# MooreThreads/LiteGS

Measured on NVIDIA H100. Metric: forward+backward views/sec @1080p 1M Gaussians, higher is better.
Workload: dtype f32

## Files before the change

### litegs_b200/csrc/sort.cu

```cuda
#include <cub/device/device_radix_sort.cuh>
#include <cub/block/block_scan.cuh>
#include <algorithm>
#include <cstdlib>
#include <cstring>
#include "common.cuh"

namespace {

constexpr int RS_THREADS = 256;
constexpr int RS_WARPS = RS_THREADS / 32;
constexpr int RS_MAXBINS = 256;

int g_sort_impl = -1;
bool g_sort_forced = false;

int sort_impl()
{
    if (g_sort_impl < 0) {
        const char* e = getenv("LGS_SORT");
        g_sort_forced = e != nullptr;
        g_sort_impl = (e != nullptr && strcmp(e, "cub") == 0) ? 0 : 1;
    }
    return g_sort_impl;
}
// ... 31 lines not shown
#pragma unroll
    for (int k = 0; k < RS_WARPS; k++) h[k][t] = 0;
    __syncthreads();
    const unsigned mask = (unsigned)nbins - 1u;
    int* hw = h[w];
    if (VEC && base + TILE <= n) {
        const uint4* v = reinterpret_cast<const uint4*>(keys + base);
#pragma unroll
        for (int j = 0; j < IPT / KPV; j++) {
            uint4 q = v[j * RS_THREADS + t];
            unsigned x[4] = { q.x, q.y, q.z, q.w };
#pragma unroll
            for (int c = 0; c < 4; c++) {
                if (sizeof(KeyT) == 2) {
                    atomicAdd(&hw[(((x[c] & 0xffffu) - bias) >> shift) & mask], 1);
                    atomicAdd(&hw[(((x[c] >> 16) - bias) >> shift) & mask], 1);
                } else {
                    atomicAdd(&hw[((x[c] - bias) >> shift) & mask], 1);
                }
            }
        }
    } else {
#pragma unroll
        for (int i = 0; i < IPT; i++) {
            int idx = base + i * RS_THREADS + t;
            if (idx < n) atomicAdd(&hw[(((unsigned)keys[idx] - bias) >> shift) & mask], 1);
        }
    }
    __syncthreads();
    if (t < nbins) {
        int c = 0;
#pragma unroll
        for (int k = 0; k < RS_WARPS; k++) c += h[k][t];
        table[(size_t)t * nblocks + blockIdx.x] = c;
    }
}

__global__ void __launch_bounds__(RS_THREADS) rs_scan_rows_kernel(int* __restrict__ table, int nblocks, int* __restrict__ totals)
{
    using BlockScan = cub::BlockScan<int, RS_THREADS>;
    __shared__ typename BlockScan::TempStorage s_scan;
    int* row = table + (size_t)blockIdx.x * nblocks;
    const int per = (nblocks + RS_THREADS - 1) / RS_THREADS;
    const int lo = min(nblocks, (int)threadIdx.x * per), hi = min(nblocks, lo + per);
    int sum = 0;
    for (int k = lo; k < hi; k++) sum += row[k];
    int pre, tot;
    BlockScan(s_scan).ExclusiveSum(sum, pre, tot);
    for (int k = lo; k < hi; k++) { int c = row[k]; row[k] = pre; pre += c; }
    if (threadIdx.x == 0) totals[blockIdx.x] = tot;
}

template <typename KeyT, int IPT, int NS>
__global__ void __launch_bounds__(RS_THREADS, IPT == 16 ? 3 : 4) rs_scatter_kernel(const KeyT* __restrict__ kin, const unsigned* __restrict__ vin,
                                                                KeyT* __restrict__ kout, unsigned* __restrict__ vout, int n, int shift,
                                                                int nbins, int nblocks, const int* __restrict__ table,
                                                                const int* __restrict__ totals, unsigned bias,
                                                                const int* __restrict__ n_dev, const unsigned* __restrict__ bias_dev)
{
    constexpr int TILE = RS_THREADS * IPT;
    static_assert(IPT % NS == 0, "the ranking rounds must tile the items of a lane");
    if (n_dev != nullptr) n = min(n, max(*n_dev, 0));
    if (bias_dev != nullptr) bias = *bias_dev;
    if ((int)blockIdx.x * TILE >= n) return;
    using BlockScan = cub::BlockScan<int, RS_THREADS>;
    __shared__ int s_cnt[RS_WARPS][RS_MAXBINS];
    __shared__ int s_gofs[RS_MAXBINS];
    __shared__ KeyT s_k[TILE];
    __shared__ unsigned s_v[TILE];
    unsigned* s_match = s_v;
    __shared__ typename BlockScan::TempStorage s_scan;
    const int t = threadIdx.x, lane = t & 31, w = t >> 5;
    const int base = blockIdx.x * TILE;
    const int nvalid = min(TILE, n - base);
    const unsigned mask = (unsigned)nbins - 1u;
    const unsigned lt = lanemask_lt();
#pragma unroll
    for (int k = 0; k < RS_WARPS; k++) s_cnt[k][t] = 0;
    for (int k = t; k < NS * RS_WARPS * nbins; k += RS_THREADS) s_match[k] = 0u;
    KeyT key[IPT];
    unsigned val[IPT];
    unsigned short rank[IPT];
#pragma unroll
    for (int i = 0; i < IPT; i++) {
        int loc = w * 32 * IPT + i * 32 + lane;
        bool valid = loc < nvalid;
        key[i] = valid ? kin[base + loc] : (KeyT)(bias - 1u);
        val[i] = valid ? vin[base + loc] : 0u;
    }
    int gdig;
    {
        int tot_d = t < nbins ? totals[t] : 0;
        BlockScan(s_scan).ExclusiveSum(tot_d, gdig);
        if (t < nbins) gdig += table[(size_t)t * nblocks + blockIdx.x];
    }
    __syncthreads();
    unsigned* mw = s_match + w * nbins;
    const int set_stride = RS_WARPS * nbins;
#pragma unroll
    for (int i0 = 0; i0 < IPT; i0 += NS) {
        unsigned d[NS];
#pragma unroll
        for (int q = 0; q < NS; q++) {
            d[q] = (((unsigned)key[i0 + q] - bias) >> shift) & mask;
            atomicOr(&mw[q * set_stride + d[q]], 1u << lane);
        }
        __syncwarp();
        unsigned own[NS];
#pragma unroll
        for (int j = 0; j < NS; j++) {
            int r = s_cnt[w][d[j]];
#pragma unroll
            for (int q = 0; q < j; q++) r += __popc(mw[q * set_stride + d[j]]);
            own[j] = mw[j * set_stride + d[j]];
            rank[i0 + j] = (unsigned short)(r + __popc(own[j] & lt));
        }
        __syncwarp();
#pragma unroll
        for (int j = 0; j < NS; j++) {
            if ((own[j] >> lane) <= 1u) {
                if (NS == 1) s_cnt[w][d[j]] = (int)rank[i0 + j] + 1;
                else atomicAdd(&s_cnt[w][d[j]], __popc(own[j]));
                mw[j * set_stride + d[j]] = 0u;
            }
        }
        __syncwarp();
    }
    __syncthreads();
    int tot = 0;
#pragma unroll
    for (int k = 0; k < RS_WARPS; k++) { int c = s_cnt[k][t]; s_cnt[k][t] = tot; tot += c; }
    int dbase;
    BlockScan(s_scan).ExclusiveSum(tot, dbase);
#pragma unroll
    for (int k = 0; k < RS_WARPS; k++) s_cnt[k][t] += dbase;
    s_gofs[t] = gdig - dbase;
    __syncthreads();
#pragma unroll
    for (int i = 0; i < IPT; i++) {
        unsigned d = (((unsigned)key[i] - bias) >> shift) & mask;
        int p = s_cnt[w][d] + rank[i];
        s_k[p] = key[i];
        s_v[p] = val[i];
    }
    __syncthreads();
#pragma unroll
    for (int i = 0; i < IPT; i++) {
        int k = i * RS_THREADS + t;
        if (k < nvalid) {
            KeyT kk = s_k[k];
            int dst = s_gofs[(((unsigned)kk - bias) >> shift) & mask] + k;
            kout[dst] = kk;
            vout[dst] = s_v[k];
        }
    }
}

constexpr unsigned LB_AGG = 1u << 30, LB_INC = 2u << 30, LB_MASK = (1u << 30) - 1u;
constexpr int RS_MAXPASS = 4;

struct GhistArgs { int shift[RS_MAXPASS]; int nbins[RS_MAXPASS]; int passes; };

template <typename KeyT, int IPT>
__global__ void __launch_bounds__(RS_THREADS) rs_ghist_kernel(const KeyT* __restrict__ keys, int n, GhistArgs A, int* __restrict__ ghist,
                                                              unsigned bias, const int* __restrict__ n_dev,
                                                              const unsigned* __restrict__ bias_dev)
{
    constexpr int TILE = RS_THREADS * IPT;
    __shared__ int h[RS_MAXPASS][RS_MAXBINS];
    const int t = threadIdx.x;
    if (n_dev != nullptr) n = min(n, max(*n_dev, 0));
    if (bias_dev != nullptr) bias = *bias_dev;
    const int base = blockIdx.x * TILE;
    if (base >= n) return;
    for (int p = 0; p < A.passes; p++) h[p][t] = 0;
    __syncthreads();
#pragma unroll
    for (int i = 0; i < IPT; i++) {
        const int idx = base + i * RS_THREADS + t;
        if (idx < n) {
            const unsigned k = (unsigned)keys[idx] - bias;
            for (int p = 0; p < A.passes; p++) atomicAdd(&h[p][(k >> A.shift[p]) & (unsigned)(A.nbins[p] - 1)], 1);
        }
    }
    __syncthreads();
    for (int p = 0; p < A.passes; p++)
        if (t < A.nbins[p] && h[p][t] != 0) atomicAdd(&ghist[p * RS_MAXBINS + t], h[p][t]);
}

template <typename KeyT, int IPT>
__global__ void __launch_bounds__(RS_THREADS) rs_onesweep_kernel(const KeyT* __restrict__ kin, const unsigned* __restrict__ vin,
                                                                 KeyT* __restrict__ kout, unsigned* __restrict__ vout, int n, int shift,
                                                                 int nbins, const int* __restrict__ ghist ,
                                                                 unsigned* __restrict__ status ,
                                                                 int* __restrict__ ticket, unsigned bias, const int* __restrict__ n_dev,
                                                                 const unsigned* __restrict__ bias_dev)
{
    constexpr int TILE = RS_THREADS * IPT;
    using BlockScan = cub::BlockScan<int, RS_THREADS>;
    __shared__ int s_cnt[RS_WARPS][RS_MAXBINS];
    __shared__ int s_gofs[RS_MAXBINS];
    __shared__ KeyT s_k[TILE];
    __shared__ unsigned s_v[TILE];
    __shared__ int s_tile;
    static_assert(TILE >= RS_WARPS * RS_MAXBINS, "the match slots alias the value staging buffer");
    unsigned (*s_match)[RS_MAXBINS] = reinterpret_cast<unsigned (*)[RS_MAXBINS]>(s_v);
    __shared__ typename BlockScan::TempStorage s_scan;
    const int t = threadIdx.x, lane = t & 31, w = t >> 5;
    if (n_dev != nullptr) n = min(n, max(*n_dev, 0));
    if (bias_dev != nullptr) bias = *bias_dev;
    if (t == 0) s_tile = atomicAdd(ticket, 1);
#pragma unroll
    for (int k = 0; k < RS_WARPS; k++) { s_cnt[k][t] = 0; s_match[k][t] = 0u; }
    __syncthreads();
    const int tile = s_tile;
    const int base = tile * TILE;
    if (base >= n) return;
    const int nvalid = min(TILE, n - base);
    const unsigned mask = (unsigned)nbins - 1u;
    const unsigned lt = lanemask_lt();
    KeyT key[IPT];
    unsigned val[IPT];
    unsigned short rank[IPT];
#pragma unroll
    for (int i = 0; i < IPT; i++) {
        int loc = w * 32 * IPT + i * 32 + lane;
        bool valid = loc < nvalid;
        key[i] = valid ? kin[base + loc] : (KeyT)(bias - 1u);
        val[i] = valid ? vin[base + loc] : 0u;
    }
    int gdig;
    {
        int tot_d = t < nbins ? ghist[t] : 0;
        BlockScan(s_scan).ExclusiveSum(tot_d, gdig);
    }
    __syncthreads();
#pragma unroll
    for (int i = 0; i < IPT; i++) {
        unsigned d = (((unsigned)key[i] - bias) >> shift) & mask;
        atomicOr(&s_match[w][d], 1u << lane);
        __syncwarp();
        unsigned m = s_match[w][d];
        int r = s_cnt[w][d] + __popc(m & lt);
        rank[i] = (unsigned short)r;
        __syncwarp();
        if ((m >> lane) <= 1u) { s_cnt[w][d] = r + 1; s_match[w][d] = 0u; }
        __syncwarp();
    }
    __syncthreads();
    int tot = 0;
#pragma unroll
    for (int k = 0; k < RS_WARPS; k++) { int c = s_cnt[k][t]; s_cnt[k][t] = tot; tot += c; }
    int real = tot;
    if (t == (int)mask) real -= (TILE - nvalid);
    if (t < nbins) {
        volatile unsigned* st_ = status + (size_t)tile * nbins;
        st_[t] = LB_AGG | (unsigned)real;
        unsigned prefix = 0u;
        for (int i = tile - 1; i >= 0;) {
            const unsigned v = *((volatile unsigned*)(status + (size_t)i * nbins + t));
            const unsigned flag = v & ~LB_MASK;
            if (flag == 0u) continue;
            prefix += v & LB_MASK;
            if (flag == LB_INC) break;
            i--;
        }
        st_[t] = LB_INC | (prefix + (unsigned)real);
        gdig += (int)prefix;
    }
    int dbase;
    BlockScan(s_scan).ExclusiveSum(tot, dbase);
#pragma unroll
    for (int k = 0; k < RS_WARPS; k++) s_cnt[k][t] += dbase;
    s_gofs[t] = gdig - dbase;
    __syncthreads();
#pragma unroll
    for (int i = 0; i < IPT; i++) {
        unsigned d = (((unsigned)key[i] - bias) >> shift) & mask;
        int p = s_cnt[w][d] + rank[i];
        s_k[p] = key[i];
        s_v[p] = val[i];
    }
    __syncthreads();
#pragma unroll
    for (int i = 0; i < IPT; i++) {
        int k = i * RS_THREADS + t;
        if (k < nvalid) {
            KeyT kk = s_k[k];
            int dst = s_gofs[(((unsigned)kk - bias) >> shift) & mask] + k;
            kout[dst] = kk;
            vout[dst] = s_v[k];
        }
    }
}

struct RsPlan {
    int ipt, tile, nblocks, passes, dbits;
    size_t table_bytes, scan_bytes, total_bytes, off_scan, off_keys, off_vals;
};

inline size_t align256(size_t x) { return (x + 255) & ~(size_t)255; }

template <typename KeyT>
RsPlan rs_plan(int n, int begin_bit, int end_bit)
{
    RsPlan p;
    static const int forced_ipt = getenv("LGS_RS_IPT") ? atoi(getenv("LGS_RS_IPT")) : 0;
    p.ipt = (forced_ipt == 8 || forced_ipt == 16) ? forced_ipt : (n > (1 << 22) ? 16 : 8);
    p.tile = RS_THREADS * p.ipt;
    p.nblocks = (n + p.tile - 1) / p.tile;
    int bits = end_bit - begin_bit;
    p.passes = bits <= 0 ? 0 : (bits + 7) / 8;
    p.dbits = p.passes == 0 ? 0 : (bits + p.passes - 1) / p.passes;
    p.table_bytes = align256((size_t)RS_MAXPASS * RS_MAXBINS * p.nblocks * sizeof(int));
    p.scan_bytes = align256((RS_MAXPASS * RS_MAXBINS + 64) * sizeof(int));
    p.off_scan = p.table_bytes;
    p.off_keys = p.off_scan + p.scan_bytes;
    p.off_vals = p.off_keys + align256((size_t)n * sizeof(KeyT));
    p.total_bytes = p.off_vals + align256((size_t)n * sizeof(unsigned));
    return p;
}

bool rs_use_onesweep();
template <typename KeyT>
int rs_sort_onesweep(const KeyT* keys_in, KeyT* keys_out, const unsigned* vals_in, unsigned* vals_out, int n, int begin_bit, int end_bit,
                     unsigned bias, char* ws, cudaStream_t st, const int* n_dev, const unsigned* bias_dev);

template <typename KeyT>
int rs_sort(const KeyT* keys_in, KeyT* keys_out, const unsigned* vals_in, unsigned* vals_out, int n, int begin_bit, int end_bit,
            unsigned bias, char* ws, cudaStream_t st, const int* n_dev = nullptr, const unsigned* bias_dev = nullptr)
{
    RsPlan p = rs_plan<KeyT>(n, begin_bit, end_bit);
    if (p.passes == 0) {
        LGS_REQUIRE(n_dev == nullptr, "sort_pairs: a device-side count needs at least one pass");
        LGS_CUDA(cudaMemcpyAsync(keys_out, keys_in, (size_t)n * sizeof(KeyT), cudaMemcpyDeviceToDevice, st));
        LGS_CUDA(cudaMemcpyAsync(vals_out, vals_in, (size_t)n * sizeof(unsigned), cudaMemcpyDeviceToDevice, st));
        return LGS_OK;
    }
    if (rs_use_onesweep())
        return rs_sort_onesweep<KeyT>(keys_in, keys_out, vals_in, vals_out, n, begin_bit, end_bit, bias, ws, st, n_dev, bias_dev);
    int* table = (int*)ws;
    int* totals = (int*)(ws + p.off_scan);
    KeyT* ktmp = (KeyT*)(ws + p.off_keys);
    unsigned* vtmp = (unsigned*)(ws + p.off_vals);
    const KeyT* ksrc = keys_in;
    const unsigned* vsrc = vals_in;
    int bit = begin_bit;
    for (int pass = 0; pass < p.passes; pass++) {
        int dbits = min(p.dbits, end_bit - bit);
        int nbins = 1 << dbits;
        bool to_out = ((p.passes - 1 - pass) & 1) == 0;
        KeyT* kdst = to_out ? keys_out : ktmp;
        unsigned* vdst = to_out ? vals_out : vtmp;
        const bool vec = ((uintptr_t)ksrc & 15) == 0;
        lgs_with_flags([&](auto ipt16, auto v) {
            rs_hist_kernel<KeyT, ipt16 ? 16 : 8, v><<<p.nblocks, RS_THREADS, 0, st>>>(ksrc, n, bit, nbins, p.nblocks, table, bias, n_dev,
                                                                                     bias_dev);
            return LGS_OK;
        }, p.ipt == 16, vec);
        LGS_CHECK_LAUNCH("rs_hist_kernel");
        rs_scan_rows_kernel<<<nbins, RS_THREADS, 0, st>>>(table, p.nblocks, totals);
        LGS_CHECK_LAUNCH("rs_scan_rows_kernel");
        static const int rank_cap = getenv("LGS_RS_RANK") ? atoi(getenv("LGS_RS_RANK")) : 2;
        int ns = 1;
        while (ns < 4 && ns * 2 <= rank_cap && ns * 2 * RS_WARPS * nbins <= p.tile) ns *= 2;
        lgs_with_flags([&](auto ipt16, auto ns4, auto ns2) {
            rs_scatter_kernel<KeyT, ipt16 ? 16 : 8, ns4 ? 4 : ns2 ? 2 : 1><<<p.nblocks, RS_THREADS, 0, st>>>(
                ksrc, vsrc, kdst, vdst, n, bit, nbins, p.nblocks, table, totals, bias, n_dev, bias_dev);
            return LGS_OK;
        }, p.ipt == 16, ns == 4, ns == 2);
        LGS_CHECK_LAUNCH("rs_scatter_kernel");
        ksrc = kdst; vsrc = vdst;
        bit += dbits;
    }
    return LGS_OK;
}

int g_rs_onesweep = -1;
bool rs_use_onesweep()
{
    if (g_rs_onesweep < 0) {
        const char* e = getenv("LGS_RS");
        g_rs_onesweep = (e != nullptr && e[0] == 'o') ? 1 : 0;
    }
    return g_rs_onesweep == 1;
}

template <typename KeyT>
int rs_sort_onesweep(const KeyT* keys_in, KeyT* keys_out, const unsigned* vals_in, unsigned* vals_out, int n, int begin_bit, int end_bit,
                     unsigned bias, char* ws, cudaStream_t st, const int* n_dev, const unsigned* bias_dev)
{
    RsPlan p = rs_plan<KeyT>(n, begin_bit, end_bit);
    unsigned* status = (unsigned*)ws;
    int* ghist = (int*)(ws + p.off_scan);
    int* tickets = ghist + RS_MAXPASS * RS_MAXBINS;
    KeyT* ktmp = (KeyT*)(ws + p.off_keys);
    unsigned* vtmp = (unsigned*)(ws + p.off_vals);
    GhistArgs A;
    A.passes = p.passes;
    size_t status_words = 0;
    int bit = begin_bit;
    for (int pass = 0; pass < p.passes; pass++) {
        int dbits = min(p.dbits, end_bit - bit);
        A.shift[pass] = bit; A.nbins[pass] = 1 << dbits;
        status_words += (size_t)p.nblocks * A.nbins[pass];
        bit += dbits;
    }
    LGS_CUDA(cudaMemsetAsync(status, 0, status_words * sizeof(unsigned), st));
    LGS_CUDA(cudaMemsetAsync(ghist, 0, (RS_MAXPASS * RS_MAXBINS + 64) * sizeof(int), st));
    lgs_with_flags([&](auto ipt16) {
        rs_ghist_kernel<KeyT, ipt16 ? 16 : 8><<<p.nblocks, RS_THREADS, 0, st>>>(keys_in, n, A, ghist, bias, n_dev, bias_dev);
        return LGS_OK;
    }, p.ipt == 16);
    LGS_CHECK_LAUNCH("rs_ghist_kernel");
    const KeyT* ksrc = keys_in;
    const unsigned* vsrc = vals_in;
    size_t soff = 0;
    for (int pass = 0; pass < p.passes; pass++) {
        bool to_out = ((p.passes - 1 - pass) & 1) == 0;
        KeyT* kdst = to_out ? keys_out : ktmp;
        unsigned* vdst = to_out ? vals_out : vtmp;
        lgs_with_flags([&](auto ipt16) {
            rs_onesweep_kernel<KeyT, ipt16 ? 16 : 8><<<p.nblocks, RS_THREADS, 0, st>>>(ksrc, vsrc, kdst, vdst, n, A.shift[pass],
                A.nbins[pass], ghist + pass * RS_MAXBINS, status + soff, tickets + pass, bias, n_dev, bias_dev);
            return LGS_OK;
        }, p.ipt == 16);
        LGS_CHECK_LAUNCH("rs_onesweep_kernel");
        soff += (size_t)p.nblocks * A.nbins[pass];
        ksrc = kdst; vsrc = vdst;
    }
    return LGS_OK;
}

template <typename KeyT>
size_t sort_workspace_bytes(int n, int max_bits)
{
    size_t cubb = 0;
    cub::DeviceRadixSort::SortPairs<KeyT, unsigned>(nullptr, cubb, nullptr, nullptr, nullptr, nullptr, n, 0, max_bits);
    size_t own = rs_plan<KeyT>(n, 0, max_bits).total_bytes;
    return std::max(cubb, own) + 256;
}

template <typename KeyT>
int sort_pairs(const char* who, const KeyT* keys_in, KeyT* keys_out, const unsigned* vals_in, unsigned* vals_out, int n, int begin_bit,
               int end_bit, unsigned bias, void* workspace, size_t workspace_bytes, void* stream)
{
    if (n <= 0) return LGS_OK;
    LGS_REQUIRE(begin_bit >= 0 && end_bit >= begin_bit && end_bit <= (int)(8 * sizeof(KeyT)), "%s: bad bit range [%d, %d)", who, begin_bit,
                end_bit);
    char* ws = (char*)(((uintptr_t)workspace + 255) & ~(uintptr_t)255);
    size_t need;
    const int impl = sort_impl_for(n, end_bit - begin_bit, bias);
    if (impl == 0) {
        if (bias != 0u) { begin_bit = 0; end_bit = 8 * (int)sizeof(KeyT); }
        need = 0;
        cub::DeviceRadixSort::SortPairs<KeyT, unsigned>(nullptr, need, nullptr, nullptr, nullptr, nullptr, n, begin_bit, end_bit);
    } else {
        need = rs_plan<KeyT>(n, begin_bit, end_bit).total_bytes;
    }
    if (workspace == nullptr || workspace_bytes < need + 256) {
        lgs_set_error("%s: workspace of %zu bytes needed, %zu given", who, need + 256, workspace_bytes);
        return LGS_ERR_WORKSPACE;
    }
    if (impl == 0) {
        LGS_CUDA(cub::DeviceRadixSort::SortPairs<KeyT, unsigned>(ws, need, keys_in, keys_out, vals_in, vals_out, n, begin_bit, end_bit,
                                                                 (cudaStream_t)stream));
        return LGS_OK;
    }
    return rs_sort<KeyT>(keys_in, keys_out, vals_in, vals_out, n, begin_bit, end_bit, bias, ws, (cudaStream_t)stream);
}

}

extern "C" int lgs_set_sort_impl(int impl)
{
    LGS_REQUIRE(impl == -1 || impl == 0 || impl == 1, "set_sort_impl: %d is not -1 (unforced), 0 (cub) or 1 (lgs)", impl);
    g_sort_impl = impl;
    g_sort_forced = impl >= 0;
    return LGS_OK;
}

extern "C" int lgs_set_radix_form(int onesweep)
{
    g_rs_onesweep = onesweep ? 1 : 0;
    return LGS_OK;
}

extern "C" int lgs_sort_pairs_u32_workspace_bytes(int n, size_t* bytes)
{
    *bytes = sort_workspace_bytes<unsigned>(n < 1 ? 1 : n, 32);
    return LGS_OK;
}

extern "C" int lgs_sort_pairs_u32(const unsigned* keys_in, unsigned* keys_out, const unsigned* vals_in, unsigned* vals_out, int n,
                                  int begin_bit, int end_bit, void* workspace, size_t workspace_bytes, void* stream)
{
    return sort_pairs<unsigned>("sort_pairs_u32", keys_in, keys_out, vals_in, vals_out, n, begin_bit, end_bit, 0u, workspace,
                                workspace_bytes, stream);
}

extern "C" int lgs_sort_pairs_u32_rebased(const unsigned* keys_in, unsigned* keys_out, const unsigned* vals_in, unsigned* vals_out, int n,
                                          unsigned bias, int end_bit, void* workspace, size_t workspace_bytes, void* stream)
{
    return sort_pairs<unsigned>("sort_pairs_u32_rebased", keys_in, keys_out, vals_in, vals_out, n, 0, end_bit, bias, workspace,
                                workspace_bytes, stream);
}

extern "C" int lgs_sort_pairs_u16_workspace_bytes(int n, size_t* bytes)
{
    *bytes = sort_workspace_bytes<unsigned short>(n < 1 ? 1 : n, 16);
    return LGS_OK;
}

extern "C" int lgs_sort_pairs_u16(const unsigned short* keys_in, unsigned short* keys_out, const unsigned* vals_in, unsigned* vals_out,
                                  int n, int begin_bit, int end_bit, void* workspace, size_t workspace_bytes, void* stream)
{
    return sort_pairs<unsigned short>("sort_pairs_u16", keys_in, keys_out, vals_in, vals_out, n, begin_bit, end_bit, 0u, workspace,
                                      workspace_bytes, stream);
}

extern "C" int lgs_sort_pairs_u32_dev(const unsigned* keys_in, unsigned* keys_out, const unsigned* vals_in, unsigned* vals_out,
                                      int capacity, const int* n_dev, const unsigned* bias_dev, int end_bit, void* workspace,
                                      size_t workspace_bytes, void* stream)
{
    if (capacity <= 0) return LGS_OK;
    LGS_REQUIRE(n_dev != nullptr && end_bit >= 1 && end_bit <= 32, "sort_pairs_u32_dev: bad arguments (end_bit %d)", end_bit);
    char* ws = (char*)(((uintptr_t)workspace + 255) & ~(uintptr_t)255);
    size_t need = rs_plan<unsigned>(capacity, 0, end_bit).total_bytes;
    if (workspace == nullptr || workspace_bytes < need + 256) {
        lgs_set_error("sort_pairs_u32_dev: workspace of %zu bytes needed, %zu given", need + 256, workspace_bytes);
        return LGS_ERR_WORKSPACE;
    }
    return rs_sort<unsigned>(keys_in, keys_out, vals_in, vals_out, capacity, 0, end_bit, 0u, ws, (cudaStream_t)stream, n_dev, bias_dev);
}

extern "C" int lgs_sort_pairs_u16_dev(const unsigned short* keys_in, unsigned short* keys_out, const unsigned* vals_in,
                                      unsigned* vals_out, int capacity, const int* n_dev, int begin_bit, int end_bit, void* workspace,
// ... 31 lines not shown
```

### profiles/microbench/dev_count_bench.py

```python
import ctypes
import sys, os
sys.path.insert(0, os.path.dirname(os.path.dirname(os.path.dirname(os.path.abspath(__file__)))))
import torch
from litegs_b200 import _lib

dev = torch.device("cuda:0")
st = lambda: torch.cuda.current_stream().cuda_stream
P = lambda t: t.data_ptr()


def timeit(fn, n=30):
    for _ in range(5):
        fn()
    torch.cuda.synchronize()
    e0 = torch.cuda.Event(enable_timing=True); e1 = torch.cuda.Event(enable_timing=True)
    e0.record()
    for _ in range(n):
        fn()
    e1.record(); torch.cuda.synchronize()
    return e0.elapsed_time(e1) / n * 1000.0


D = 10_897_674
for cap in (D, int(D * 1.3) + 65536):
    keys = torch.randint(1, 16201, (cap,), device=dev, dtype=torch.int32).to(torch.int16)
    vals = torch.arange(cap, device=dev, dtype=torch.int32)
    ko, vo = torch.empty_like(keys), torch.empty_like(vals)
    nb = ctypes.c_size_t(0)
    _lib.call("lgs_sort_pairs_u16_workspace_bytes", cap, ctypes.byref(nb))
    ws = torch.empty(nb.value, dtype=torch.uint8, device=dev)
    ndev = torch.tensor([D], dtype=torch.int32, device=dev)
    t_host = timeit(lambda: _lib.call("lgs_sort_pairs_u16", P(keys), P(ko), P(vals), P(vo), D, 0, 14, P(ws), ctypes.c_size_t(nb.value), st()))
    t_dev = timeit(lambda: _lib.call("lgs_sort_pairs_u16_dev", P(keys), P(ko), P(vals), P(vo), cap, P(ndev), 0, 14, P(ws), ctypes.c_size_t(nb.value), st()))
    print(f"tile sort D={D} capacity={cap}: host count {t_host:.1f} us, device count {t_dev:.1f} us")

N = 1_000_064
k32 = torch.randint(0, 1 << 24, (N,), device=dev, dtype=torch.int32)
v32 = torch.arange(N, device=dev, dtype=torch.int32)
ko, vo = torch.empty_like(k32), torch.empty_like(v32)
nb = ctypes.c_size_t(0)
_lib.call("lgs_sort_pairs_u32_workspace_bytes", N, ctypes.byref(nb))
ws = torch.empty(nb.value, dtype=torch.uint8, device=dev)
ndev = torch.tensor([984_960], dtype=torch.int32, device=dev)
bias = torch.zeros(1, dtype=torch.int32, device=dev)
t_host = timeit(lambda: _lib.call("lgs_sort_pairs_u32_rebased", P(k32), P(ko), P(v32), P(vo), 984_960, 0, 24, P(ws), ctypes.c_size_t(nb.value), st()))
t_dev = timeit(lambda: _lib.call("lgs_sort_pairs_u32_dev", P(k32), P(ko), P(v32), P(vo), N, P(ndev), P(bias), 24, P(ws), ctypes.c_size_t(nb.value), st()))
print(f"depth sort N=984960 (capacity {N}): host count {t_host:.1f} us, device count {t_dev:.1f} us")
cnt = torch.randint(0, 20, (N,), device=dev, dtype=torch.int32)
out = torch.empty(N, dtype=torch.int32, device=dev)
nb2 = ctypes.c_size_t(0)
_lib.call("lgs_scan_gathered_workspace_bytes", N, ctypes.byref(nb2))
ws2 = torch.empty(nb2.value, dtype=torch.uint8, device=dev)
order = torch.randperm(N, device=dev).to(torch.int32)
t_host = timeit(lambda: _lib.call("lgs_scan_gathered", P(cnt), P(order), 984_960, P(out), P(ws2), ctypes.c_size_t(nb2.value), st()))
t_dev = timeit(lambda: _lib.call("lgs_scan_gathered_dev", P(cnt), P(order), N, P(ndev), P(out), P(ws2), ctypes.c_size_t(nb2.value), st()))
print(f"gathered scan: host count {t_host:.1f} us, device count {t_dev:.1f} us")

D4 = 71_700_532
keys = torch.randint(1, 64801, (D4,), device=dev, dtype=torch.int32).to(torch.int16)
vals = torch.arange(D4, device=dev, dtype=torch.int32)
ko, vo = torch.empty_like(keys), torch.empty_like(vals)
nb = ctypes.c_size_t(0)
_lib.call("lgs_sort_pairs_u16_workspace_bytes", D4, ctypes.byref(nb))
ws = torch.empty(nb.value, dtype=torch.uint8, device=dev)
t = timeit(lambda: _lib.call("lgs_sort_pairs_u16", P(keys), P(ko), P(vals), P(vo), D4, 0, 16, P(ws), ctypes.c_size_t(nb.value), st()), n=10)
print(f"C4 tile sort D={D4}, 16 bits, LGS_RS_IPT={os.environ.get('LGS_RS_IPT', 'default')}, LGS_SORT={os.environ.get('LGS_SORT', 'lgs')}: {t:.1f} us "
      f"= {D4 * (2 + 2 * 12) / t / 1e6:.2f} TB/s of algorithmic traffic")
```

Baseline: 947.4.

## Rework onesweep radix sort: multi-round ranking, vectorized histogram, overlapped lookback

Moves the scatter kernel's ranking, staging and write phases into shared device helpers, and makes the onesweep kernel rank several items per round (NS) instead of one at a time with per-item warp syncs. The global histogram kernel becomes a grid-stride loop over 16-byte vector loads that merges runs of equal digits before each shared atomic. The onesweep kernel now publishes its tile's aggregate, then does shared-memory staging before the decoupled lookback so the lookback wait overlaps that work. It also adds a full-tile fast path for loads and makes onesweep selection depend on n. The cost is more shared memory for match slots, a changed launch-bounds occupancy, and a dispatch heuristic that is not fully visible here.

New measurement: 972.9 (median of 6 runs). 1.03x the previous value.

```diff
diff --git a/litegs_b200/csrc/sort.cu b/litegs_b200/csrc/sort.cu
--- a/litegs_b200/csrc/sort.cu
+++ b/litegs_b200/csrc/sort.cu
@@ -107,6 +107,71 @@
 }
 
 template <typename KeyT, int IPT, int NS>
+__device__ __forceinline__ void rs_rank_tile(const KeyT (&key)[IPT], unsigned short (&rank)[IPT], int* cnt, unsigned* match, int set_stride,
+                                             int shift, unsigned mask, unsigned bias, int lane, unsigned lt)
+{
+    static_assert(IPT % NS == 0, "the ranking rounds must tile the items of a lane");
+#pragma unroll
+    for (int i0 = 0; i0 < IPT; i0 += NS) {
+        unsigned d[NS];
+#pragma unroll
+        for (int q = 0; q < NS; q++) {
+            d[q] = (((unsigned)key[i0 + q] - bias) >> shift) & mask;
+            atomicOr(&match[q * set_stride + d[q]], 1u << lane);
+        }
+        __syncwarp();
+        unsigned own[NS];
+#pragma unroll
+        for (int j = 0; j < NS; j++) {
+            int r = cnt[d[j]];
+#pragma unroll
+            for (int q = 0; q < j; q++) r += __popc(match[q * set_stride + d[j]]);
+            own[j] = match[j * set_stride + d[j]];
+            rank[i0 + j] = (unsigned short)(r + __popc(own[j] & lt));
+        }
+        __syncwarp();
+#pragma unroll
+        for (int j = 0; j < NS; j++) {
+            if ((own[j] >> lane) <= 1u) {
+                if (NS == 1) cnt[d[j]] = (int)rank[i0 + j] + 1;
+                else atomicAdd(&cnt[d[j]], __popc(own[j]));
+                match[j * set_stride + d[j]] = 0u;
+            }
+        }
+        __syncwarp();
+    }
+}
+
+template <typename KeyT, int IPT>
+__device__ __forceinline__ void rs_stage_tile(const KeyT (&key)[IPT], const unsigned (&val)[IPT], const unsigned short (&rank)[IPT],
+                                              const int* cnt, KeyT* s_k, unsigned* s_v, int shift, unsigned mask, unsigned bias)
+{
+#pragma unroll
+    for (int i = 0; i < IPT; i++) {
+        unsigned d = (((unsigned)key[i] - bias) >> shift) & mask;
+        int p = cnt[d] + rank[i];
+        s_k[p] = key[i];
+        s_v[p] = val[i];
+    }
+}
+
+template <typename KeyT, int IPT>
+__device__ __forceinline__ void rs_write_tile(const int* gofs, const KeyT* s_k, const unsigned* s_v, KeyT* __restrict__ kout,
+                                              unsigned* __restrict__ vout, int nvalid, int shift, unsigned mask, unsigned bias, int t)
+{
+#pragma unroll
+    for (int i = 0; i < IPT; i++) {
+        int k = i * RS_THREADS + t;
+        if (k < nvalid) {
+            KeyT kk = s_k[k];
+            int dst = gofs[(((unsigned)kk - bias) >> shift) & mask] + k;
+            kout[dst] = kk;
+            vout[dst] = s_v[k];
+        }
+    }
+}
+
+template <typename KeyT, int IPT, int NS>
 __global__ void __launch_bounds__(RS_THREADS, IPT == 16 ? 3 : 4) rs_scatter_kernel(const KeyT* __restrict__ kin, const unsigned* __restrict__ vin,
                                                                 KeyT* __restrict__ kout, unsigned* __restrict__ vout, int n, int shift,
                                                                 int nbins, int nblocks, const int* __restrict__ table,
@@ -114,7 +179,6 @@
                                                                 const int* __restrict__ n_dev, const unsigned* __restrict__ bias_dev)
 {
     constexpr int TILE = RS_THREADS * IPT;
-    static_assert(IPT % NS == 0, "the ranking rounds must tile the items of a lane");
     if (n_dev != nullptr) n = min(n, max(*n_dev, 0));
     if (bias_dev != nullptr) bias = *bias_dev;
     if ((int)blockIdx.x * TILE >= n) return;
@@ -150,37 +214,7 @@
         if (t < nbins) gdig += table[(size_t)t * nblocks + blockIdx.x];
     }
     __syncthreads();
-    unsigned* mw = s_match + w * nbins;
-    const int set_stride = RS_WARPS * nbins;
-#pragma unroll
-    for (int i0 = 0; i0 < IPT; i0 += NS) {
-        unsigned d[NS];
-#pragma unroll
-        for (int q = 0; q < NS; q++) {
-            d[q] = (((unsigned)key[i0 + q] - bias) >> shift) & mask;
-            atomicOr(&mw[q * set_stride + d[q]], 1u << lane);
-        }
-        __syncwarp();
-        unsigned own[NS];
-#pragma unroll
-        for (int j = 0; j < NS; j++) {
-            int r = s_cnt[w][d[j]];
-#pragma unroll
-            for (int q = 0; q < j; q++) r += __popc(mw[q * set_stride + d[j]]);
-            own[j] = mw[j * set_stride + d[j]];
-            rank[i0 + j] = (unsigned short)(r + __popc(own[j] & lt));
-        }
-        __syncwarp();
-#pragma unroll
-        for (int j = 0; j < NS; j++) {
-            if ((own[j] >> lane) <= 1u) {
-                if (NS == 1) s_cnt[w][d[j]] = (int)rank[i0 + j] + 1;
-                else atomicAdd(&s_cnt[w][d[j]], __popc(own[j]));
-                mw[j * set_stride + d[j]] = 0u;
-            }
-        }
-        __syncwarp();
-    }
+    rs_rank_tile<KeyT, IPT, NS>(key, rank, s_cnt[w], s_match + w * nbins, RS_WARPS * nbins, shift, mask, bias, lane, lt);
     __syncthreads();
     int tot = 0;
 #pragma unroll
@@ -191,24 +225,9 @@
     for (int k = 0; k < RS_WARPS; k++) s_cnt[k][t] += dbase;
     s_gofs[t] = gdig - dbase;
     __syncthreads();
-#pragma unroll
-    for (int i = 0; i < IPT; i++) {
-        unsigned d = (((unsigned)key[i] - bias) >> shift) & mask;
-        int p = s_cnt[w][d] + rank[i];
-        s_k[p] = key[i];
-        s_v[p] = val[i];
-    }
-    __syncthreads();
-#pragma unroll
-    for (int i = 0; i < IPT; i++) {
-        int k = i * RS_THREADS + t;
-        if (k < nvalid) {
-            KeyT kk = s_k[k];
-            int dst = s_gofs[(((unsigned)kk - bias) >> shift) & mask] + k;
-            kout[dst] = kk;
-            vout[dst] = s_v[k];
-        }
-    }
+    rs_stage_tile<KeyT, IPT>(key, val, rank, s_cnt[w], s_k, s_v, shift, mask, bias);
+    __syncthreads();
+    rs_write_tile<KeyT, IPT>(s_gofs, s_k, s_v, kout, vout, nvalid, shift, mask, bias, t);
 }
 
 constexpr unsigned LB_AGG = 1u << 30, LB_INC = 2u << 30, LB_MASK = (1u << 30) - 1u;
@@ -216,57 +235,102 @@
 
 struct GhistArgs { int shift[RS_MAXPASS]; int nbins[RS_MAXPASS]; int passes; };
 
-template <typename KeyT, int IPT>
+template <typename KeyT>
+__device__ __forceinline__ void rs_ghist_add(int (*h)[RS_MAXBINS], const GhistArgs& A, unsigned k, unsigned bias)
+{
+    k -= bias;
+#pragma unroll
+    for (int p = 0; p < RS_MAXPASS; p++)
+        if (p < A.passes) atomicAdd(&h[p][(k >> A.shift[p]) & (unsigned)(A.nbins[p] - 1)], 1);
+}
+
+template <typename KeyT>
+__device__ __forceinline__ void rs_ghist_vec(int (*h)[RS_MAXBINS], const GhistArgs& A, uint4 q, unsigned bias)
+{
+    constexpr int KPV = 16 / (int)sizeof(KeyT);
+    const unsigned x[4] = { q.x, q.y, q.z, q.w };
+    unsigned k[KPV];
+#pragma unroll
+    for (int c = 0; c < 4; c++) {
+        if (sizeof(KeyT) == 2) { k[2 * c] = (x[c] & 0xffffu) - bias; k[2 * c + 1] = (x[c] >> 16) - bias; }
+        else k[c] = x[c] - bias;
+    }
+#pragma unroll
+    for (int p = 0; p < RS_MAXPASS; p++) {
+        if (p >= A.passes) break;
+        const unsigned m = (unsigned)(A.nbins[p] - 1);
+        const int sh = A.shift[p];
+        unsigned cur = (k[0] >> sh) & m;
+        int run = 1;
+#pragma unroll
+        for (int i = 1; i < KPV; i++) {
+            const unsigned d = (k[i] >> sh) & m;
+            if (d == cur) { run++; continue; }
+            atomicAdd(&h[p][cur], run);
+            cur = d;
+            run = 1;
+        }
+        atomicAdd(&h[p][cur], run);
+    }
+}
+
+template <typename KeyT>
 __global__ void __launch_bounds__(RS_THREADS) rs_ghist_kernel(const KeyT* __restrict__ keys, int n, GhistArgs A, int* __restrict__ ghist,
                                                               unsigned bias, const int* __restrict__ n_dev,
                                                               const unsigned* __restrict__ bias_dev)
 {
-    constexpr int TILE = RS_THREADS * IPT;
+    constexpr int KPV = 16 / (int)sizeof(KeyT);
     __shared__ int h[RS_MAXPASS][RS_MAXBINS];
     const int t = threadIdx.x;
     if (n_dev != nullptr) n = min(n, max(*n_dev, 0));
     if (bias_dev != nullptr) bias = *bias_dev;
-    const int base = blockIdx.x * TILE;
-    if (base >= n) return;
-    for (int p = 0; p < A.passes; p++) h[p][t] = 0;
-    __syncthreads();
-#pragma unroll
-    for (int i = 0; i < IPT; i++) {
-        const int idx = base + i * RS_THREADS + t;
-        if (idx < n) {
-            const unsigned k = (unsigned)keys[idx] - bias;
-            for (int p = 0; p < A.passes; p++) atomicAdd(&h[p][(k >> A.shift[p]) & (unsigned)(A.nbins[p] - 1)], 1);
-        }
+#pragma unroll
+    for (int p = 0; p < RS_MAXPASS; p++) h[p][t] = 0;
+    __syncthreads();
+    const int head = min(n, (int)(((16 - ((uintptr_t)keys & 15)) & 15) / sizeof(KeyT)));
+    const int nvec = (n - head) / KPV;
+    const uint4* v = reinterpret_cast<const uint4*>(keys + head);
+    const int stride = gridDim.x * RS_THREADS;
+    for (int j = blockIdx.x * RS_THREADS + t; j < nvec; j += 2 * stride) {
+        const uint4 q0 = v[j];
+        const bool two = j + stride < nvec;
+        const uint4 q1 = two ? v[j + stride] : q0;
+        rs_ghist_vec<KeyT>(h, A, q0, bias);
+        if (two) rs_ghist_vec<KeyT>(h, A, q1, bias);
+    }
+    if (blockIdx.x == 0) {
+        for (int i = t; i < head; i += RS_THREADS) rs_ghist_add<KeyT>(h, A, (unsigned)keys[i], bias);
+        for (int i = head + nvec * KPV + t; i < n; i += RS_THREADS) rs_ghist_add<KeyT>(h, A, (unsigned)keys[i], bias);
     }
     __syncthreads();
     for (int p = 0; p < A.passes; p++)
         if (t < A.nbins[p] && h[p][t] != 0) atomicAdd(&ghist[p * RS_MAXBINS + t], h[p][t]);
 }
 
-template <typename KeyT, int IPT>
-__global__ void __launch_bounds__(RS_THREADS) rs_onesweep_kernel(const KeyT* __restrict__ kin, const unsigned* __restrict__ vin,
-                                                                 KeyT* __restrict__ kout, unsigned* __restrict__ vout, int n, int shift,
-                                                                 int nbins, const int* __restrict__ ghist ,
-                                                                 unsigned* __restrict__ status ,
-                                                                 int* __restrict__ ticket, unsigned bias, const int* __restrict__ n_dev,
-                                                                 const unsigned* __restrict__ bias_dev)
+template <typename KeyT, int IPT, int NS>
+__global__ void __launch_bounds__(RS_THREADS, (sizeof(KeyT) == 2 && IPT <= 16) ? 3 : 2)
+rs_onesweep_kernel(const KeyT* __restrict__ kin, const unsigned* __restrict__ vin, KeyT* __restrict__ kout, unsigned* __restrict__ vout,
+                   int n, int shift, int nbins, const int* __restrict__ ghist ,
+                   unsigned* __restrict__ status , int stride, int* __restrict__ ticket, unsigned bias,
+                   const int* __restrict__ n_dev, const unsigned* __restrict__ bias_dev)
 {
     constexpr int TILE = RS_THREADS * IPT;
     using BlockScan = cub::BlockScan<int, RS_THREADS>;
     __shared__ int s_cnt[RS_WARPS][RS_MAXBINS];
     __shared__ int s_gofs[RS_MAXBINS];
+    __shared__ int s_look[RS_MAXBINS];
     __shared__ KeyT s_k[TILE];
     __shared__ unsigned s_v[TILE];
     __shared__ int s_tile;
-    static_assert(TILE >= RS_WARPS * RS_MAXBINS, "the match slots alias the value staging buffer");
-    unsigned (*s_match)[RS_MAXBINS] = reinterpret_cast<unsigned (*)[RS_MAXBINS]>(s_v);
+    unsigned* s_match = s_v;
     __shared__ typename BlockScan::TempStorage s_scan;
     const int t = threadIdx.x, lane = t & 31, w = t >> 5;
     if (n_dev != nullptr) n = min(n, max(*n_dev, 0));
     if (bias_dev != nullptr) bias = *bias_dev;
     if (t == 0) s_tile = atomicAdd(ticket, 1);
 #pragma unroll
-    for (int k = 0; k < RS_WARPS; k++) { s_cnt[k][t] = 0; s_match[k][t] = 0u; }
+    for (int k = 0; k < RS_WARPS; k++) s_cnt[k][t] = 0;
+    for (int k = t; k < NS * RS_WARPS * nbins; k += RS_THREADS) s_match[k] = 0u;
     __syncthreads();
     const int tile = s_tile;
     const int base = tile * TILE;
@@ -277,76 +341,60 @@
     KeyT key[IPT];
     unsigned val[IPT];
     unsigned short rank[IPT];
-#pragma unroll
-    for (int i = 0; i < IPT; i++) {
-        int loc = w * 32 * IPT + i * 32 + lane;
-        bool valid = loc < nvalid;
-        key[i] = valid ? kin[base + loc] : (KeyT)(bias - 1u);
-        val[i] = valid ? vin[base + loc] : 0u;
+    if (nvalid == TILE) {
+#pragma unroll
+        for (int i = 0; i < IPT; i++) {
+            const int loc = w * 32 * IPT + i * 32 + lane;
+            key[i] = kin[base + loc];
+            val[i] = vin[base + loc];
+        }
+    } else {
+#pragma unroll
+        for (int i = 0; i < IPT; i++) {
+            const int loc = w * 32 * IPT + i * 32 + lane;
+            const bool valid = loc < nvalid;
+            key[i] = valid ? kin[base + loc] : (KeyT)(bias - 1u);
+            val[i] = valid ? vin[base + loc] : 0u;
+        }
     }
     int gdig;
     {
         int tot_d = t < nbins ? ghist[t] : 0;
         BlockScan(s_scan).ExclusiveSum(tot_d, gdig);
     }
-    __syncthreads();
-#pragma unroll
-    for (int i = 0; i < IPT; i++) {
-        unsigned d = (((unsigned)key[i] - bias) >> shift) & mask;
-        atomicOr(&s_match[w][d], 1u << lane);
-        __syncwarp();
-        unsigned m = s_match[w][d];
-        int r = s_cnt[w][d] + __popc(m & lt);
-        rank[i] = (unsigned short)r;
-        __syncwarp();
-        if ((m >> lane) <= 1u) { s_cnt[w][d] = r + 1; s_match[w][d] = 0u; }
-        __syncwarp();
-    }
+    rs_rank_tile<KeyT, IPT, NS>(key, rank, s_cnt[w], s_match + w * nbins, RS_WARPS * nbins, shift, mask, bias, lane, lt);
     __syncthreads();
     int tot = 0;
 #pragma unroll
     for (int k = 0; k < RS_WARPS; k++) { int c = s_cnt[k][t]; s_cnt[k][t] = tot; tot += c; }
-    int real = tot;
-    if (t == (int)mask) real -= (TILE - nvalid);
     if (t < nbins) {
-        volatile unsigned* st_ = status + (size_t)tile * nbins;
-        st_[t] = LB_AGG | (unsigned)real;
+        const int real = t == (int)mask ? tot - (TILE - nvalid) : tot;
+        *(volatile unsigned*)(status + (size_t)tile * stride + t) = (tile == 0 ? LB_INC : LB_AGG) | (unsigned)real;
+        s_look[t] = real;
+    }
+    int dbase;
+    BlockScan(s_scan).ExclusiveSum(tot, dbase);
+#pragma unroll
+    for (int k = 0; k < RS_WARPS; k++) s_cnt[k][t] += dbase;
+    __syncthreads();
+    rs_stage_tile<KeyT, IPT>(key, val, rank, s_cnt[w], s_k, s_v, shift, mask, bias);
+    if (t < nbins) {
         unsigned prefix = 0u;
         for (int i = tile - 1; i >= 0;) {
-            const unsigned v = *((volatile unsigned*)(status + (size_t)i * nbins + t));
+            const unsigned v = *((const volatile unsigned*)(status + (size_t)i * stride + t));
             const unsigned flag = v & ~LB_MASK;
             if (flag == 0u) continue;
             prefix += v & LB_MASK;
             if (flag == LB_INC) break;
             i--;
         }
-        st_[t] = LB_INC | (prefix + (unsigned)real);
-        gdig += (int)prefix;
-    }
-    int dbase;
-    BlockScan(s_scan).ExclusiveSum(tot, dbase);
-#pragma unroll
-    for (int k = 0; k < RS_WARPS; k++) s_cnt[k][t] += dbase;
-    s_gofs[t] = gdig - dbase;
-    __syncthreads();
-#pragma unroll
-    for (int i = 0; i < IPT; i++) {
-        unsigned d = (((unsigned)key[i] - bias) >> shift) & mask;
-        int p = s_cnt[w][d] + rank[i];
-        s_k[p] = key[i];
-        s_v[p] = val[i];
-    }
-    __syncthreads();
-#pragma unroll
-    for (int i = 0; i < IPT; i++) {
-        int k = i * RS_THREADS + t;
-        if (k < nvalid) {
-            KeyT kk = s_k[k];
-            int dst = s_gofs[(((unsigned)kk - bias) >> shift) & mask] + k;
-            kout[dst] = kk;
-            vout[dst] = s_v[k];
-        }
-    }
+        if (tile > 0) *(volatile unsigned*)(status + (size_t)tile * stride + t) = LB_INC | (prefix + (unsigned)s_look[t]);
+        s_look[t] = (int)prefix;
+    }
+    __syncthreads();
+    if (t < nbins) s_gofs[t] = gdig + s_look[t] - dbase;
+    __syncthreads();
+    rs_write_tile<KeyT, IPT>(s_gofs, s_k, s_v, kout, vout, nvalid, shift, mask, bias, t);
 }
 
 struct RsPlan {
@@ -376,7 +424,7 @@
     return p;
 }
 
-bool rs_use_onesweep();
+bool rs_use_onesweep(int n);
 template <typename KeyT>
 int rs_sort_onesweep(const KeyT* keys_in, KeyT* keys_out, const unsigned* vals_in, unsigned* vals_out, int n, int begin_bit, int end_bit,
                      unsigned bias, char* ws, cudaStream_t st, const int* n_dev, const unsigned* bias_dev);
@@ -392,7 +440,7 @@
         LGS_CUDA(cudaMemcpyAsync(vals_out, vals_in, (size_t)n * sizeof(unsigned), cudaMemcpyDeviceToDevice, st));
         return LGS_OK;
     }
-    if (rs_use_onesweep())
+    if (rs_use_onesweep(n))
         return rs_sort_onesweep<KeyT>(keys_in, keys_out, vals_in, vals_out, n, begin_bit, end_bit, bias, ws, st, n_dev, bias_dev);
     int* table = (int*)ws;
     int* totals = (int*)(ws + p.off_scan);
@@ -431,14 +479,14 @@
     return LGS_OK;
 }
 
-int g_rs_onesweep = -1;
-bool rs_use_onesweep()
-{
-    if (g_rs_onesweep < 0) {
+int g_rs_onesweep = -2;
+bool rs_use_onesweep(int n)
+{
+    if (g_rs_onesweep == -2) {
         const char* e = getenv("LGS_RS");
-        g_rs_onesweep = (e != nullptr && e[0] == 'o') ? 1 : 0;
-    }
-    return g_rs_onesweep == 1;
+        g_rs_onesweep = e == nullptr ? -1 : e[0] == 'o' ? 1 : 0;
+    }
+    return g_rs_onesweep < 0 ? n > (1 << 22) : g_rs_onesweep == 1;
 }
 
 template <typename KeyT>
@@ -446,6 +494,7 @@
                      unsigned bias, char* ws, cudaStream_t st, const int* n_dev, const unsigned* bias_dev)
 {
     RsPlan p = rs_plan<KeyT>(n, begin_bit, end_bit);
+    if (p.ipt == 16 && sizeof(KeyT) == 2) { p.ipt = 24; p.tile = RS_THREADS * p.ipt; p.nblocks = (n + p.tile - 1) / p.tile; }
     unsigned* status = (unsigned*)ws;
     int* ghist = (int*)(ws + p.off_scan);
     int* tickets = ghist + RS_MAXPASS * RS_MAXBINS;
@@ -463,10 +512,16 @@
     }
     LGS_CUDA(cudaMemsetAsync(status, 0, status_words * sizeof(unsigned), st));
     LGS_CUDA(cudaMemsetAsync(ghist, 0, (RS_MAXPASS * RS_MAXBINS + 64) * sizeof(int), st));
-    lgs_with_flags([&](auto ipt16) {
-        rs_ghist_kernel<KeyT, ipt16 ? 16 : 8><<<p.nblocks, RS_THREADS, 0, st>>>(keys_in, n, A, ghist, bias, n_dev, bias_dev);
-        return LGS_OK;
-    }, p.ipt == 16);
+    static int ghist_grid = 0;
+    if (ghist_grid == 0) {
+        int dev = 0, sms = 0;
+        LGS_CUDA(cudaGetDevice(&dev));
+        LGS_CUDA(cudaDeviceGetAttribute(&sms, cudaDevAttrMultiProcessorCount, dev));
+        ghist_grid = 8 * std::max(sms, 1);
+    }
+    const int kpv = 16 / (int)sizeof(KeyT);
+    const int grid = std::max(1, std::min(ghist_grid, (n / kpv + RS_THREADS - 1) / RS_THREADS));
+    rs_ghist_kernel<KeyT><<<grid, RS_THREADS, 0, st>>>(keys_in, n, A, ghist, bias, n_dev, bias_dev);
     LGS_CHECK_LAUNCH("rs_ghist_kernel");
     const KeyT* ksrc = keys_in;
     const unsigned* vsrc = vals_in;
@@ -475,11 +530,18 @@
         bool to_out = ((p.passes - 1 - pass) & 1) == 0;
         KeyT* kdst = to_out ? keys_out : ktmp;
         unsigned* vdst = to_out ? vals_out : vtmp;
-        lgs_with_flags([&](auto ipt16) {
-            rs_onesweep_kernel<KeyT, ipt16 ? 16 : 8><<<p.nblocks, RS_THREADS, 0, st>>>(ksrc, vsrc, kdst, vdst, n, A.shift[pass],
-                A.nbins[pass], ghist + pass * RS_MAXBINS, status + soff, tickets + pass, bias, n_dev, bias_dev);
-            return LGS_OK;
-        }, p.ipt == 16);
+        const bool ns2 = p.ipt != 24 && 2 * RS_WARPS * A.nbins[pass] <= p.tile;
+        auto launch = [&](auto ipt_c) {
+            constexpr int IPT = decltype(ipt_c)::value;
+            lgs_with_flags([&](auto two) {
+                rs_onesweep_kernel<KeyT, IPT, two ? 2 : 1><<<p.nblocks, RS_THREADS, 0, st>>>(ksrc, vsrc, kdst, vdst, n, A.shift[pass],
+                    A.nbins[pass], ghist + pass * RS_MAXBINS, status + soff, A.nbins[pass], tickets + pass, bias, n_dev, bias_dev);
+                return LGS_OK;
+            }, ns2);
+        };
+        if (p.ipt == 8) launch(std::integral_constant<int, 8>{});
+        else if (p.ipt == 16) launch(std::integral_constant<int, 16>{});
+        else if constexpr (sizeof(KeyT) == 2) launch(std::integral_constant<int, 24>{});
         LGS_CHECK_LAUNCH("rs_onesweep_kernel");
         soff += (size_t)p.nblocks * A.nbins[pass];
         ksrc = kdst; vsrc = vdst;
@@ -537,7 +599,7 @@
 
 extern "C" int lgs_set_radix_form(int onesweep)
 {
-    g_rs_onesweep = onesweep ? 1 : 0;
+    g_rs_onesweep = onesweep < 0 ? -1 : onesweep ? 1 : 0;
     return LGS_OK;
 }
 
diff --git a/profiles/microbench/dev_count_bench.py b/profiles/microbench/dev_count_bench.py
--- a/profiles/microbench/dev_count_bench.py
+++ b/profiles/microbench/dev_count_bench.py
@@ -1,38 +1,153 @@
+import argparse
 import ctypes
-import sys, os
+import os
+import subprocess
+import sys
+
 sys.path.insert(0, os.path.dirname(os.path.dirname(os.path.dirname(os.path.abspath(__file__)))))
 import torch
-from litegs_b200 import _lib
+from litegs_b200 import _lib, pipeline, scene
+
+ap = argparse.ArgumentParser()
+ap.add_argument("--reps", type=int, default=50)
+ap.add_argument("--skip-c4", action="store_true")
+args = ap.parse_args()
 
 dev = torch.device("cuda:0")
 st = lambda: torch.cuda.current_stream().cuda_stream
 P = lambda t: t.data_ptr()
+REPS = max(50, args.reps)
+FORMS = [("passes", 1, 0), ("onesweep", 1, 1), ("cub", 0, 0)]
 
 
-def timeit(fn, n=30):
+def card():
+    try:
+        q = subprocess.run(["nvidia-smi", "--query-gpu=name,power.limit,clocks.max.sm", "--format=csv,noheader"], capture_output=True,
+                           text=True, timeout=30).stdout.strip().splitlines()[0]
+    except Exception as e:
+        q = f"{torch.cuda.get_device_name(0)}, power limit unknown ({e})"
+    return q
+
+
+def median(xs):
+    xs = sorted(xs)
+    return xs[len(xs) // 2]
+
+
+def time_call(fn, reps=REPS):
     for _ in range(5):
         fn()
     torch.cuda.synchronize()
-    e0 = torch.cuda.Event(enable_timing=True); e1 = torch.cuda.Event(enable_timing=True)
-    e0.record()
-    for _ in range(n):
+    ev = [(torch.cuda.Event(enable_timing=True), torch.cuda.Event(enable_timing=True)) for _ in range(reps)]
+    for e0, e1 in ev:
+        e0.record()
         fn()
-    e1.record(); torch.cuda.synchronize()
-    return e0.elapsed_time(e1) / n * 1000.0
+        e1.record()
+    torch.cuda.synchronize()
+    return median([e0.elapsed_time(e1) * 1000.0 for e0, e1 in ev])
 
 
-D = 10_897_674
-for cap in (D, int(D * 1.3) + 65536):
-    keys = torch.randint(1, 16201, (cap,), device=dev, dtype=torch.int32).to(torch.int16)
-    vals = torch.arange(cap, device=dev, dtype=torch.int32)
-    ko, vo = torch.empty_like(keys), torch.empty_like(vals)
-    nb = ctypes.c_size_t(0)
-    _lib.call("lgs_sort_pairs_u16_workspace_bytes", cap, ctypes.byref(nb))
-    ws = torch.empty(nb.value, dtype=torch.uint8, device=dev)
-    ndev = torch.tensor([D], dtype=torch.int32, device=dev)
-    t_host = timeit(lambda: _lib.call("lgs_sort_pairs_u16", P(keys), P(ko), P(vals), P(vo), D, 0, 14, P(ws), ctypes.c_size_t(nb.value), st()))
-    t_dev = timeit(lambda: _lib.call("lgs_sort_pairs_u16_dev", P(keys), P(ko), P(vals), P(vo), cap, P(ndev), 0, 14, P(ws), ctypes.c_size_t(nb.value), st()))
-    print(f"tile sort D={D} capacity={cap}: host count {t_host:.1f} us, device count {t_dev:.1f} us")
+def time_kernels(fn, reps=REPS):
+    from torch.profiler import ProfilerActivity, profile
+    for _ in range(5):
+        fn()
+    torch.cuda.synchronize()
+    with profile(activities=[ProfilerActivity.CUDA]) as prof:
+        for _ in range(reps):
+            fn()
+        torch.cuda.synchronize()
+    evs = [e for e in prof.events() if e.device_type == torch.autograd.DeviceType.CUDA]
+    evs.sort(key=lambda e: e.time_range.start)
+    per = len(evs) // reps
+    if per == 0 or per * reps != len(evs):
+        return [("(activities did not divide into calls)", float("nan"))]
+    out = []
+    for j in range(per):
+        name = evs[j].name
+        short = name.split("<")[0].split("(")[0].replace("void ", "").split("::")[-1].strip() or name[:40]
+        if "memset" in name.lower():
+            short = "memset"
+        out.append((short, median([evs[r * per + j].time_range.elapsed_us() for r in range(reps)])))
+    return out
+
+
+def set_form(impl, form):
+    _lib.call("lgs_set_sort_impl", impl)
+    _lib.call("lgs_set_radix_form", form)
+
+
+def unforce():
+    _lib.call("lgs_set_sort_impl", -1)
+    _lib.call("lgs_set_radix_form", 0)
+
+
+def sort_bytes(n, key_bytes, passes):
+    return n * (key_bytes + passes * 2 * (key_bytes + 4))
+
+
+def line(what, us, nbytes):
+    print(f"  {what:<58s} {us:9.1f} us  {nbytes / 1e6:8.1f} MB  {nbytes / us / 1e3:7.1f} GB/s", flush=True)
+
+
+def c2_pairs():
+    H, W, tile = 1080, 1920, (8, 16)
+    p = scene.make_scene(1_000_000, sh_degree=3, seed=0)
+    keys_p = ("xyz", "scale", "rot", "sh_0", "sh_rest", "opacity")
+    Pm = {k: torch.from_numpy(p[k]).to(dev) for k in keys_p}
+    co, ce = (torch.from_numpy(p[k]).to(dev) for k in ("cluster_origin", "cluster_extend"))
+    cam = {k: torch.from_numpy(v).to(dev) for k, v in scene.make_camera(0, 64, W, H).items()}
+    _, stv, _ = pipeline.render_view_forward(Pm, co, ce, cam["frustumplane"], cam["view"], cam["proj"], 3, (H, W), tile)
+    D = int(stv.n_pairs)
+    ws = pipeline.ViewWorkspace(Pm, (H, W), tile, int(D * 1.3) + 65536, 24, use_graphs=False)
+    ws.forward(Pm, co, ce, cam, 3)
+    torch.cuda.synchronize()
+    assert int(ws.vparams[1]) == D, (int(ws.vparams[1]), D)
+    return ws.keys[:D].clone(), ws.vals[:D].clone(), D, ws.ntile
+
+
+print(f"card: {card()}", flush=True)
+keys, vals, D, ntile = c2_pairs()
+bits = ntile.bit_length()
+cap = int(D * 1.3) + 65536
+print(f"C2 tile sort: D = {D} emitted pairs (u16 keys, u32 values), {ntile} tiles -> bits [0, {bits}), capacity {cap}", flush=True)
+kin = torch.zeros(cap, dtype=torch.int16, device=dev)
+vin = torch.zeros(cap, dtype=torch.int32, device=dev)
+kin[:D], vin[:D] = keys, vals
+ko, vo = torch.empty_like(kin), torch.empty_like(vin)
+nb = ctypes.c_size_t(0)
+_lib.call("lgs_sort_pairs_u16_workspace_bytes", cap, ctypes.byref(nb))
+ws = torch.empty(nb.value, dtype=torch.uint8, device=dev)
+ndev = torch.tensor([D], dtype=torch.int32, device=dev)
+passes = (bits + 7) // 8
+B = sort_bytes(D, 2, passes)
+host = lambda: _lib.call("lgs_sort_pairs_u16", P(kin), P(ko), P(vin), P(vo), D, 0, bits, P(ws), ctypes.c_size_t(nb.value), st())
+devc = lambda: _lib.call("lgs_sort_pairs_u16_dev", P(kin), P(ko), P(vin), P(vo), cap, P(ndev), 0, bits, P(ws), ctypes.c_size_t(nb.value), st())
+ref = None
+for name, impl, form in FORMS:
+    set_form(impl, form)
+    try:
+        entries = [("host count", host)] + ([] if name == "cub" else [(f"_dev, capacity {cap}", devc)])
+        for ename, fn in entries:
+            us = time_call(fn)
+            line(f"{name:<9s} {ename}", us, B)
+            for kname, kus in time_kernels(fn):
+                print(f"      {kname:<40s} {kus:8.1f} us")
+            torch.cuda.synchronize()
+            got = (ko[:D].clone(), vo[:D].clone())
+            if ref is None:
+                ref = got
+            same = torch.equal(got[0], ref[0]) and torch.equal(got[1], ref[1])
+            print(f"      output identical to the first form's: {same}")
+    finally:
+        unforce()
+
+ranges = torch.empty((1, ntile + 2), dtype=torch.int32, device=dev)
+ks = ref[0].clone()
+rng_fn = lambda: _lib.call("lgs_tile_range_u16", P(ks), 1, D, ntile, 1, P(ranges), st())
+us = time_call(rng_fn)
+line("tile_range_bsearch (u16, host count)", us, 2 * D)
+for kname, kus in time_kernels(rng_fn):
+    print(f"      {kname:<40s} {kus:8.1f} us")
 
 N = 1_000_064
 k32 = torch.randint(0, 1 << 24, (N,), device=dev, dtype=torch.int32)
@@ -43,26 +158,41 @@
 ws = torch.empty(nb.value, dtype=torch.uint8, device=dev)
 ndev = torch.tensor([984_960], dtype=torch.int32, device=dev)
 bias = torch.zeros(1, dtype=torch.int32, device=dev)
-t_host = timeit(lambda: _lib.call("lgs_sort_pairs_u32_rebased", P(k32), P(ko), P(v32), P(vo), 984_960, 0, 24, P(ws), ctypes.c_size_t(nb.value), st()))
-t_dev = timeit(lambda: _lib.call("lgs_sort_pairs_u32_dev", P(k32), P(ko), P(v32), P(vo), N, P(ndev), P(bias), 24, P(ws), ctypes.c_size_t(nb.value), st()))
-print(f"depth sort N=984960 (capacity {N}): host count {t_host:.1f} us, device count {t_dev:.1f} us")
+B = sort_bytes(984_960, 4, 3)
+for name, impl, form in FORMS[:2]:
+    set_form(impl, form)
+    try:
+        t_host = time_call(lambda: _lib.call("lgs_sort_pairs_u32_rebased", P(k32), P(ko), P(v32), P(vo), 984_960, 0, 24, P(ws),
+                                             ctypes.c_size_t(nb.value), st()))
+        t_dev = time_call(lambda: _lib.call("lgs_sort_pairs_u32_dev", P(k32), P(ko), P(v32), P(vo), N, P(ndev), P(bias), 24, P(ws),
+                                            ctypes.c_size_t(nb.value), st()))
+    finally:
+        unforce()
+    line(f"depth sort {name} N=984960 (capacity {N}) host count", t_host, B)
+    line(f"depth sort {name} N=984960 (capacity {N}) device count", t_dev, B)
 cnt = torch.randint(0, 20, (N,), device=dev, dtype=torch.int32)
 out = torch.empty(N, dtype=torch.int32, device=dev)
 nb2 = ctypes.c_size_t(0)
 _lib.call("lgs_scan_gathered_workspace_bytes", N, ctypes.byref(nb2))
 ws2 = torch.empty(nb2.value, dtype=torch.uint8, device=dev)
 order = torch.randperm(N, device=dev).to(torch.int32)
-t_host = timeit(lambda: _lib.call("lgs_scan_gathered", P(cnt), P(order), 984_960, P(out), P(ws2), ctypes.c_size_t(nb2.value), st()))
-t_dev = timeit(lambda: _lib.call("lgs_scan_gathered_dev", P(cnt), P(order), N, P(ndev), P(out), P(ws2), ctypes.c_size_t(nb2.value), st()))
+t_host = time_call(lambda: _lib.call("lgs_scan_gathered", P(cnt), P(order), 984_960, P(out), P(ws2), ctypes.c_size_t(nb2.value), st()))
+t_dev = time_call(lambda: _lib.call("lgs_scan_gathered_dev", P(cnt), P(order), N, P(ndev), P(out), P(ws2), ctypes.c_size_t(nb2.value), st()))
 print(f"gathered scan: host count {t_host:.1f} us, device count {t_dev:.1f} us")
 
-D4 = 71_700_532
-keys = torch.randint(1, 64801, (D4,), device=dev, dtype=torch.int32).to(torch.int16)
-vals = torch.arange(D4, device=dev, dtype=torch.int32)
-ko, vo = torch.empty_like(keys), torch.empty_like(vals)
-nb = ctypes.c_size_t(0)
-_lib.call("lgs_sort_pairs_u16_workspace_bytes", D4, ctypes.byref(nb))
-ws = torch.empty(nb.value, dtype=torch.uint8, device=dev)
-t = timeit(lambda: _lib.call("lgs_sort_pairs_u16", P(keys), P(ko), P(vals), P(vo), D4, 0, 16, P(ws), ctypes.c_size_t(nb.value), st()), n=10)
-print(f"C4 tile sort D={D4}, 16 bits, LGS_RS_IPT={os.environ.get('LGS_RS_IPT', 'default')}, LGS_SORT={os.environ.get('LGS_SORT', 'lgs')}: {t:.1f} us "
-      f"= {D4 * (2 + 2 * 12) / t / 1e6:.2f} TB/s of algorithmic traffic")
+if not args.skip_c4:
+    D4 = 71_700_532
+    keys = torch.randint(1, 64801, (D4,), device=dev, dtype=torch.int32).to(torch.int16)
+    vals = torch.arange(D4, device=dev, dtype=torch.int32)
+    ko, vo = torch.empty_like(keys), torch.empty_like(vals)
+    nb = ctypes.c_size_t(0)
+    _lib.call("lgs_sort_pairs_u16_workspace_bytes", D4, ctypes.byref(nb))
+    ws = torch.empty(nb.value, dtype=torch.uint8, device=dev)
+    for name, impl, form in FORMS + [("automatic", -1, 0)]:
+        set_form(impl, form)
+        try:
+            t = time_call(lambda: _lib.call("lgs_sort_pairs_u16", P(keys), P(ko), P(vals), P(vo), D4, 0, 16, P(ws), ctypes.c_size_t(nb.value),
+                                            st()), reps=max(20, REPS // 2))
+        finally:
+            unforce()
+        line(f"C4 tile sort {name} D={D4}, 16 bits", t, sort_bytes(D4, 2, 2))
```
